# Lennart0HU/Master-Thesis-Deep-Reinforcement-Learning-DDPG-in-Home-Energy-Management

Hardware: AMD Instinct MI355X
Metric: env-steps/sec (higher is better)
Workload: dtype f32; 1 GPU; 65536 parallel shems_LU1 envs per GPU, Charger98 synthetic train table (4320 rows), 72-step episodes, mode=train; envs_per_gpu=65536, episode_len=72, mode=train

## Files before the change

master-thesis-deep-reinforcement-learning-ddpg-in-home-energy-management_amd/csrc/shems_ddpg.hip:

```cpp
#include <hip/hip_runtime.h>

#include <cstring>
#include <type_traits>

#include "philox.h"
#include "shems_internal.h"
#include "shems_adam.h"

namespace shems {

typedef float f32x16 __attribute__((ext_vector_type(16)));

#ifdef SHEMS_STAMP
__device__ unsigned long long *g_stamps = nullptr;
#define STAMP(region, i) do { if (threadIdx.x == 0 && g_stamps) { unsigned long long *sp_ = g_stamps + ((((size_t)(region) * 1024 + blockIdx.x) * 16 + (i)) * 2); \
        sp_[0] = __builtin_amdgcn_s_memtime(); sp_[1] = __builtin_amdgcn_s_memrealtime(); } } while (0)
#else
#define STAMP(region, i)
#endif

constexpr int BP = 128;
constexpr int H1N = SHEMS_L1, H2N = SHEMS_L2;
constexpr int SIN = 9, AIN = 2, CIN = 11;
constexpr int NT = 16;
// ... 25 lines not shown
constexpr int64_t WS_DAP = WS_IDX + BP;
constexpr int64_t WS_FW3C = WS_DAP + NT16 * AIN * BP;
constexpr int64_t WS_FW3A = WS_FW3C + 512;
constexpr int64_t WS_FB3 = WS_FW3A + 1024;
constexpr int64_t WS_W1T = WS_FB3 + 8;
constexpr int64_t WS_EA1 = WS_W1T + 4 * 12 * 256;
constexpr int64_t WS_SLOT0 = WS_EA1 + NQ * H1N * BP;
constexpr int64_t SL_H2 = 0;
constexpr int64_t SL_P3 = SL_H2 + H2N * BP;
constexpr int64_t SL_EP = SL_P3 + NT * 2 * BP;
constexpr int64_t SL_SIZE = SL_EP + NQ * H1N * BP;
enum { SLOT_ACTOR_T = 0, SLOT_CRITIC_T = 1, SLOT_CRITIC = 2, SLOT_ACTOR = 3, SLOT_CRITIC2 = 4, N_SLOTS = 5 };
static_assert(WS_W1T % 4 == 0 && WS_SLOT0 % 4 == 0 && SL_SIZE % 4 == 0, "16-byte aligned blocks");
__host__ __device__ inline float *w1t_of(float *ws, int net) { return ws + WS_W1T + (int64_t)net * 12 * 256; }
constexpr int64_t WS_SYNC = WS_SLOT0 + N_SLOTS * SL_SIZE;
constexpr int64_t WS_FLOATS = WS_SYNC + 96;
static_assert(WS_FLOATS == kTpWsFloats, "shems_internal.h states the workspace size for shems_gupd.hip");

__host__ __device__ inline float *slot(float *ws, int s) { return ws + WS_SLOT0 + (int64_t)s * SL_SIZE; }

template <int CTRL, int ROW_MASK>
__device__ __forceinline__ float dpp_add(float x)
{
    const int y = __builtin_amdgcn_update_dpp(0, __builtin_bit_cast(int, x), CTRL, ROW_MASK, 0xF, false);
    return x + __builtin_bit_cast(float, y);
}
__device__ __forceinline__ float wave_sum(float x)
{
    x = dpp_add<0xB1, 0xF>(x);
    x = dpp_add<0x4E, 0xF>(x);
    x = dpp_add<0x141, 0xF>(x);
// ... 230 lines not shown
    }
}

struct FwdJob {
    const float *w1t;
    const float *P;
    int in;
    int out;
    int which;
    XSrc x;
    float *H2;
    float *P3;
    const float *d3q;
    float *DAP;
    const float *W2t;
};
struct FwdArgs { FwdJob job[3]; int64_t gstride; int prep; PrepArgs pa; };
__device__ __forceinline__ void gshift(FwdJob &J, int64_t off)
{
    J.w1t = gsh(J.w1t, off); J.P = gsh(J.P, off); gshift(J.x, off); J.H2 = gsh(J.H2, off); J.P3 = gsh(J.P3, off);
    J.d3q = gsh(J.d3q, off); J.DAP = gsh(J.DAP, off);
}

template <bool QG> struct FwdShape {
    static constexpr int WST = QG ? 36 : 32;
    static constexpr int LDS = (256 * WST + W1K * 32 + W1K * W1C + 256 + 4 * 16 * 64 + 4 * 2 * 32 + (QG ? 32 * 32 + 4 * 2 * 32 : 0)) * 4;
};

template <int IN, int PREP, bool QG, bool CLONE = false, bool TILED = false>
__device__ __forceinline__ void fwd_body(const FwdJob &J, float *smem, const PrepArgs *pa, int bx, int job)
{
    typedef FwdShape<QG> SH;
    constexpr int WST = SH::WST;
    float *Wc = smem;
    float *xs = Wc + 256 * WST;
    float *w1 = xs + W1K * 32;
    float *ep = w1 + W1K * W1C;
    float *xch = ep + 256;
    float *pp = xch + 4 * 16 * 64;
    float *Mt = pp + 4 * 2 * 32;
    float *red = Mt + 32 * 32;
    const int tid = threadIdx.x, lane = tid & 63, wave = tid >> 6, li = lane & 31, lh = lane >> 5;
    constexpr int kMTiles = BP / 32;
    constexpr int kRegion = PREP == 1 ? 0 : PREP == 0 ? 1 : 3;
    (void)kRegion;
    STAMP(kRegion, 0);
    if (PREP == 1 && bx >= NT * kMTiles) {
        if (job != 0) return;
        const int duty = bx - NT * kMTiles;
        const shems_ddpg &d = pa->d;
        if (duty == 0) {
            if (tid < BP) {
                PrepRegs pr;
                prep_load<CLONE>(*pa, tid, 0, true, pr);
// ... 105 lines not shown
    STAMP(kRegion, 5);
    {
        float xv[4][4], eb[4], e0[4], e1[4];
#pragma unroll
        for (int q = 0; q < 4; ++q)
#pragma unroll
            for (int r = 0; r < 4; ++r) xv[q][r] = xch[(q * 16 + 4 * wave + r) * 64 + lane];
#pragma unroll
        for (int r = 0; r < 4; ++r) {
            const int nl = r + 8 * wave + 4 * lh;
            eb[r] = ep[nl * 3]; e0[r] = ep[nl * 3 + 1]; e1[r] = ep[nl * 3 + 2];
        }
        __builtin_amdgcn_sched_barrier(0);
        const int m = mbase + li;
        float p0 = 0.0f, p1 = 0.0f;
#pragma unroll
        for (int r = 0; r < 4; ++r) {
            const int nl = r + 8 * wave + 4 * lh, n = n0 + nl;
            const float sum = ((xv[0][r] + xv[1][r]) + xv[2][r]) + xv[3][r];
            const float h = n < H2N ? fmaxf(sum + eb[r], 0.0f) : 0.0f;
            if (J.H2 && n < H2N) J.H2[n * BP + m] = h;
            p0 = fmaf(h, e0[r], p0);
            p1 = fmaf(h, e1[r], p1);
            if (QG) Mt[nl * 32 + li] = h > 0.0f ? e0[r] * d3q : 0.0f;
        }
        p0 += __shfl_xor(p0, 32, 64);
        p1 += __shfl_xor(p1, 32, 64);
        if (lh == 0) { pp[(wave * 2 + 0) * 32 + li] = p0; pp[(wave * 2 + 1) * 32 + li] = p1; }
    }
    __syncthreads();
    STAMP(kRegion, 6);
    if (tid < 64) {
        const int o = tid >> 5, c = tid & 31;
        const float s = ((pp[(0 * 2 + o) * 32 + c] + pp[(1 * 2 + o) * 32 + c]) + pp[(2 * 2 + o) * 32 + c]) + pp[(3 * 2 + o) * 32 + c];
        J.P3[(ntile * 2 + o) * BP + mbase + c] = s;
    }
    if (!QG) return;
    STAMP(kRegion, 7);
    {
        float bq[16];
#pragma unroll
        for (int u = 0; u < 16; ++u) bq[u] = Mt[(2 * u + lh) * 32 + li];
        float da0 = 0.0f, da1 = 0.0f;
#pragma unroll
        for (int q = 0; q < 2; ++q) {
            const int kb = 64 * wave + 32 * q;
            float aq[16], wa0[16], wa1[16];
#pragma unroll
            for (int u = 0; u < 16; ++u) aq[u] = Wc[(kb + li) * WST + 2 * u + lh];
#pragma unroll
// ... 214 lines not shown
    const int job = A.prep == 1 ? (int)blockIdx.x / kPerJob : 0, bx = (int)blockIdx.x - job * kPerJob;
    FwdJob J = job == 0 ? A.job[0] : job == 1 ? A.job[1] : A.job[2];
    gshift(J, blockIdx.z * A.gstride);
    if (A.prep == 1) {
        PrepArgs pa = A.pa;
        gshift(pa.d, blockIdx.z * A.gstride); gshift(pa.ring, blockIdx.z * A.gstride); pa.seed += blockIdx.z;
        if (J.in == SIN) fwd_body<SIN, 1, false>(J, smem, &pa, bx, job); else fwd_body<CIN, 1, false>(J, smem, &pa, bx, job);
        return;
    }
    qg16_body(J, smem, bx);
}

struct EJob {
    const float *P;
    int in, out, col;
    const float *H2;
    float *EP;
    const float *W2t;
};
struct MidArgs { FwdJob fwd; EJob e[3]; int64_t gstride; int nfwd; };
constexpr int E_LDS = (NQW * BP + 32 * (NQW + 1) + NQW) * 4;

template <bool TILED = false>
__device__ __forceinline__ void e_body(const EJob &E, int b, float *smem)
{
    float *Bt = smem;
    float *At = Bt + NQW * BP;
    float *w3s = At + 32 * (NQW + 1);
    const int tid = threadIdx.x, lane = tid & 63, wave = tid >> 6, li = lane & 31, lh = lane >> 5;
    const int kt = b >> 3, nq = b & 7, nb = nq * NQW;
    const int mcol = tid & 127, half = tid >> 7;
    const float *__restrict__ P = E.P;
    const float *__restrict__ W2p = P + off_w2(E.in);
    STAMP(1, 0);
    float hv[32], wvp[8], w3v = 0.0f;
#pragma unroll
    for (int u = 0; u < 32; ++u) hv[u] = E.H2[min(nb + 2 * u + half, H2N - 1) * BP + mcol];
#pragma unroll
    for (int u = 0; u < 8; ++u) {
        const int e = u * 256 + tid, kl = e >> 6, nl = e & 63, k = kt * 32 + kl, n = nb + nl;
        if constexpr (TILED) wvp[u] = E.W2t[w2t_idx(k, n)];
        else wvp[u] = W2p[(int64_t)min(k, H1N - 1) * H2N + min(n, H2N - 1)];
    }
    w3v = P[off_w3(E.in) + min(nb + min(tid, NQW - 1), H2N - 1) * E.out + E.col];
    if (tid < NQW) w3s[tid] = nb + tid < H2N ? w3v : 0.0f;
    STAMP(1, 1);
    __syncthreads();
    STAMP(1, 2);
#pragma unroll
    for (int u = 0; u < 32; ++u) {
        const int nl = 2 * u + half;
        Bt[nl * BP + mcol] = hv[u] > 0.0f ? w3s[nl] : 0.0f;
    }
#pragma unroll
    for (int u = 0; u < 8; ++u) {
        const int e = u * 256 + tid, kl = e >> 6, nl = e & 63;
        At[kl * (NQW + 1) + nl] = wvp[u];
    }
    STAMP(1, 3);
    __syncthreads();
    STAMP(1, 4);
    f32x16 acc;
#pragma unroll
    for (int r = 0; r < 16; ++r) acc[r] = 0.0f;
    const float *pa = At + li * (NQW + 1), *pb = Bt + wave * 32 + li;
    {
        float ac[8], bc[8], an[8], bn[8];
// ... 11 lines not shown
#pragma unroll
            for (int u = 0; u < 8; ++u) acc = __builtin_amdgcn_mfma_f32_32x32x2f32(ac[u], bc[u], acc, 0, 0, 0);
#pragma unroll
            for (int u = 0; u < 8; ++u) { ac[u] = an[u]; bc[u] = bn[u]; }
        }
    }
    STAMP(1, 5);
    const int m = wave * 32 + li;
    float *D = E.EP + (int64_t)nq * H1N * BP;
#pragma unroll
    for (int r = 0; r < 16; ++r) {
        const int k = kt * 32 + (r & 3) + 8 * (r >> 2) + 4 * lh;
        if (k < H1N) D[k * BP + m] = acc[r];
    }
    STAMP(1, 6);
}

__global__ __launch_bounds__(256) __attribute__((amdgpu_waves_per_eu(1, 2))) void k_mid(MidArgs A)
{
    extern __shared__ __attribute__((aligned(16))) float smem[];
    const int64_t off = blockIdx.z * A.gstride;
    if ((int)blockIdx.x < A.nfwd) {
        FwdJob J = A.fwd;
        gshift(J, off);
        fwd_body<CIN, 0, false>(J, smem, nullptr, (int)blockIdx.x, 0);
        return;
    }
    const int e = (int)blockIdx.x - A.nfwd;
    const int set = e / (KT * NQ);
    EJob E = set == 0 ? A.e[0] : set == 1 ? A.e[1] : A.e[2];
    E.P = gsh(E.P, off); E.H2 = gsh(E.H2, off); E.EP = gsh(E.EP, off);
    e_body(E, e % (KT * NQ), smem);
}

__device__ __forceinline__ void adam_elem(const AdamCtx &c, int i, float graw)
{
    float m = c.mt[i], v = c.vt[i], p = c.p[i], t = c.target[i];
    adam_math(c, graw, m, v, p, t);
    c.mt[i] = m; c.vt[i] = v; c.p[i] = p; c.target[i] = t;
    if (c.publish) pub_store(c.publish + i, p, true);
}
template <int N>
__device__ __forceinline__ void adam_batch(const AdamCtx &c, const int (&idx)[N], const float (&g)[N])
{
    float m[N], v[N], p[N], t[N];
#pragma unroll
// ... 65 lines not shown
    const int64_t l = blockIdx.z;
    gshift(c, l * gstride);
    c.eta = critic ? hp[l].eta_crit : hp[l].eta_act;
    c.k1 = c.eta / (1.0 - c.bp1);
    c.tau = hp[l].tau;
    const int i0 = 4 * ((int)blockIdx.x * (int)blockDim.x + (int)threadIdx.x);
    if (i0 < c.n) adam_vec4(c, i0);
}

struct HeadRegs { float v[2 * NT]; float s[4]; };
static_assert(2 * NT >= NT16, "HeadRegs.v holds the actor head's NT16 partials");
__device__ __forceinline__ void head_loss_load(const shems_ddpg &d, HeadRegs &R)
{
    const float *ws = d.ws;
    const int m = threadIdx.x & 127;
    const float *Pt = slot(d.ws, SLOT_CRITIC_T) + SL_P3, *Pc = slot(d.ws, SLOT_CRITIC) + SL_P3;
#pragma unroll
    for (int i = 0; i < NT; ++i) { R.v[i] = Pt[(i * 2) * BP + m]; R.v[NT + i] = Pc[(i * 2) * BP + m]; }
    R.s[0] = ws[WS_FB3 + 1];
    R.s[1] = ws[WS_FB3 + 0];
    R.s[2] = ws[WS_R + m];
    R.s[3] = ws[WS_DONE + m];
}
__device__ __forceinline__ void head_actor_load(const shems_ddpg &d, HeadRegs &R, bool wt = false)
{
    const float *ws = d.ws;
    const int t = threadIdx.x, o = t >> 7, m = t & 127;
#pragma unroll
    for (int p = 0; p < NT16; ++p) R.v[p] = pub_load(ws + WS_DAP + (int64_t)(p * 2 + o) * BP + m, wt);
    R.s[0] = pub_load(ws + WS_API + t, wt);
    R.s[1] = R.s[2] = R.s[3] = 0.0f;
}

__device__ __forceinline__ void head_loss(const shems_ddpg &d, const HeadRegs &R, float *d3 , float *red , bool publisher,
                                          const AdamCtx *fuse)
{
    float *ws = d.ws;
    const int t = threadIdx.x, m = t & 127;
    float dq = 0.0f, diff = 0.0f;
    if (t < BP) {
        float q2 = R.s[0], q = R.s[1];
#pragma unroll
        for (int i = 0; i < NT; ++i) { q2 += R.v[i]; q += R.v[NT + i]; }
        const float y = R.s[2] + d.gamma * (1.0f - R.s[3]) * q2;
        diff = m < d.batch ? q - y : 0.0f;
        dq = 2.0f * diff / (float)d.batch;
        if (publisher) { ws[WS_Y + m] = y; ws[WS_Q + m] = q; ws[WS_D3C + m] = dq; }
    }
    d3[t] = t < BP ? dq : 0.0f;
    if (publisher) {
        const float s1 = wave_sum(diff * diff), s2 = wave_sum(dq);
        if ((t & 63) == 0) { red[t >> 6] = s1; red[4 + (t >> 6)] = s2; }
        __syncthreads();
        if (t == 0) {
            d.losses[0] = (red[0] + red[1]) / (float)d.batch;
            const float g = red[4] + red[5];
            d.grad_critic[off_b3(CIN, 1)] = g;
            if (fuse) adam_elem(*fuse, off_b3(CIN, 1), g);
        }
// ... 66 lines not shown
            const float g0 = red[0] + red[1], g1 = red[2] + red[3];
            d.grad_actor[off_b3(SIN, 2) + 0] = g0;
            d.grad_actor[off_b3(SIN, 2) + 1] = g1;
            d.losses[1] = ((red[4] + red[5]) + (red[6] + red[7])) / (2.0f * (float)d.batch);
            if (fuse) { adam_elem(*fuse, off_b3(SIN, 2), g0); adam_elem(*fuse, off_b3(SIN, 2) + 1, g1); }
        }
    }
}

struct GradArgs {
    const float *w1t;
    const float *P;
    int in, out;
    XSrc x;
    const float *H2;
    const float *w3f;
    float *grad;
    const float *E0, *E1;
    int head;
    int fuse;
    shems_ddpg dd;
    AdamCtx c;
    int64_t gstride;
    float *w2t;
};
__device__ __forceinline__ void gshift(GradArgs &B, int64_t off)
{
    B.w1t = gsh(B.w1t, off); B.P = gsh(B.P, off); gshift(B.x, off); B.H2 = gsh(B.H2, off); B.w3f = gsh(B.w3f, off);
    B.grad = gsh(B.grad, off); B.E0 = gsh(B.E0, off); B.E1 = gsh(B.E1, off); gshift(B.dd, off); gshift(B.c, off);
}
constexpr int GR_WN = 32;
enum { GR_NTW = 512 / GR_WN, GR_NW = KT * GR_NTW, GR_NG = 16, GR_GROWS = 512 / GR_NG, GR_GU = GR_GROWS / 4, GR_NR = (H1N + 3) / 4 };

constexpr int GR_PS = BP + 4;
constexpr int GR_BT = GR_WN * GR_PS;
constexpr int GR_AT = 32 * GR_PS;
constexpr int GR_LDS = (GR_BT + GR_AT + W1K * BP + W1K * 32 + AIN * BP + 2 * 32 + 8 + GR_GROWS * 3) * 4;

__device__ __forceinline__ float d2_val(float h2, float w3a, float w3b, float d3a, float d3b)
{
    const float g = fmaf(w3b, d3b, w3a * d3a);
    return h2 > 0.0f ? g : 0.0f;
}

template <int IN, int OUT> struct L1Row { float w[IN]; float b; float e[OUT][2][NQ]; float x[2][IN]; };
template <int IN, int OUT>
__device__ __forceinline__ void l1row_load(const GradArgs &A, int k, int lane, L1Row<IN, OUT> &R)
{
#pragma unroll
    for (int j = 0; j < IN; ++j) R.w[j] = A.P[j * H1N + k];
    R.b = A.P[off_b1(IN) + k];
#pragma unroll
    for (int h = 0; h < 2; ++h) {
        const int m = lane + 64 * h;
#pragma unroll
        for (int q = 0; q < NQ; ++q) {
            R.e[0][h][q] = A.E0[((int64_t)q * H1N + k) * BP + m];
// ... 43 lines not shown
    const AdamCtx *fz = A.fuse ? &A.c : nullptr;
    const bool publisher = bx == 0;
    constexpr int kRegion = OUT == 1 ? 2 : 4;
    (void)kRegion;
    STAMP(kRegion, 0);

    if (!is_w && !is_g) {
        const int k = (bx - GR_NW - GR_NG) * 4 + wave;
        HeadRegs hr;
        L1Row<IN, OUT> R;
        l1row_load<IN, OUT>(A, min(k, H1N - 1), lane, R);
        if constexpr (CLONE) head_clone_load(A.dd, hr);
        else if (A.head == 1) head_loss_load(A.dd, hr); else head_actor_load(A.dd, hr);
        STAMP(kRegion, 1);
        if constexpr (CLONE) head_clone(A.dd, hr, d3, red, false, nullptr);
        else if (A.head == 1) head_loss(A.dd, hr, d3, red, false, nullptr); else head_actor(A.dd, hr, d3, red, false, nullptr);
        __syncthreads();
        STAMP(kRegion, 2);
        if (k >= H1N) return;
        float gout[IN + 1];
        l1row_wave<IN, OUT>(R, d3, lane, gout);
        STAMP(kRegion, 3);
        float mine = 0.0f;
#pragma unroll
        for (int j = 0; j <= IN; ++j) mine = lane == j ? gout[j] : mine;
        if (lane <= IN) {
            const int e = lane < IN ? lane * H1N + k : off_b1(IN) + k;
            A.grad[e] = mine;
            if (fz) adam_elem(*fz, e, mine);
        }
        STAMP(kRegion, 4);
        return;
    }

    constexpr int HVN = GR_WN / 2;
    constexpr int WOWN = 4;
    float hv[HVN];
    int widx[WOWN];
    [[maybe_unused]] int tidx[WOWN];
    [[maybe_unused]] AdamCtx cw;
    if constexpr (TILED) {
        cw = A.c;
        cw.mt = A.w2t; cw.vt = A.w2t + W2T_TILE; cw.p = A.w2t + 2 * W2T_TILE; cw.target = A.w2t + 3 * W2T_TILE; cw.publish = nullptr;
    }
#pragma unroll
    for (int r = 0; r < WOWN; ++r) {
        widx[r] = -1;
        if constexpr (TILED) tidx[r] = -1;
    }
    AdamRegs<WOWN> ar;
    if (is_w) {
#pragma unroll
        for (int u = 0; u < HVN; ++u) hv[u] = A.H2[min(nt * GR_WN + 2 * u + half, H2N - 1) * BP + mcol];
#pragma unroll
        for (int r = 0; r < WOWN; ++r) {
            const int k = kt * 32 + 16 * (wave >> 1) + 4 * (lane >> 4) + r, n = nt * GR_WN + 16 * (wave & 1) + (lane & 15);
            widx[r] = (k < H1N && n < H2N) ? off_w2(IN) + k * H2N + n : -1;
            if constexpr (TILED) tidx[r] = (k < H1N && n < H2N) ? w2t_idx(k, n) : -1;
        }
        if constexpr (TILED) adam_load<WOWN>(cw, tidx, ar);
        else adam_load<WOWN>(A.c, widx, ar);
    }
    XRegs<IN> xr;
    f32x4 wq = {0.f, 0.f, 0.f, 0.f};
    float w3v = 0.0f;
    const int nrow0 = is_w ? nt * GR_WN : (bx - GR_NW) * GR_GROWS;
    if (is_w) {
        build_x_load<IN>(A.x, xr);
// ... 14 lines not shown
    if constexpr (CLONE) head_clone(A.dd, hr, d3, red, publisher, fz);
    else if (A.head == 1) head_loss(A.dd, hr, d3, red, publisher, fz); else head_actor(A.dd, hr, d3, red, publisher, fz);
    if (tid < 2 * 32) w3s[tid] = (tid & 1) < OUT ? w3v : 0.0f;
    STAMP(kRegion, 1);
    __syncthreads();
    STAMP(kRegion, 2);
    const float d3a = d3[mcol], d3b = d3[BP + mcol];

    if (is_w) {
        const f32x16 t = l1_tile<32>(w1, xs, 0, wave * 32, li, lh);
        {
#pragma unroll
            for (int u = 0; u < HVN; ++u) {
                const int nl = 2 * u + half;
                const float2 w = *reinterpret_cast<const float2 *>(w3s + 2 * nl);
                Bt[nl * GR_PS + mcol] = d2_val(hv[u], w.x, w.y, d3a, d3b);
            }
        }
#pragma unroll
        for (int r = 0; r < 16; ++r) At[((r & 3) + 8 * (r >> 2) + 4 * lh) * GR_PS + wave * 32 + li] = fmaxf(t[r], 0.0f);
        STAMP(kRegion, 3);
        __syncthreads();
        STAMP(kRegion, 4);
        f32x4 blk;
        {
            const int g = lane >> 4, c = lane & 15;
            const float *pa = At + (16 * (wave >> 1) + c) * GR_PS + 4 * g, *pb = Bt + (16 * (wave & 1) + c) * GR_PS + 4 * g;
            f32x4 av[8], bv[8];
#pragma unroll
            for (int q = 0; q < 8; ++q) {
                av[q] = *reinterpret_cast<const f32x4 *>(pa + 16 * q);
// ... 27 lines not shown
        const float e0a = d3[lane], e0b = d3[64 + lane], e1a = d3[BP + lane], e1b = d3[BP + 64 + lane];
        {
            float h0[GR_GU], h1[GR_GU];
#pragma unroll
            for (int u = 0; u < GR_GU; ++u) {
                const int nc = min(g * GR_GROWS + wave + 4 * u, H2N - 1);
                h0[u] = A.H2[nc * BP + lane];
                h1[u] = A.H2[nc * BP + 64 + lane];
            }
#pragma unroll
            for (int u = 0; u < GR_GU; ++u) {
                const int rl = wave + 4 * u;
                const float2 w = *reinterpret_cast<const float2 *>(w3s + 2 * rl);
                const float s0 = wave_sum(h0[u] * e0a + h1[u] * e0b);
                const float s1 = wave_sum(h0[u] * e1a + h1[u] * e1b);
                const float sb = wave_sum(d2_val(h0[u], w.x, w.y, e0a, e1a) + d2_val(h1[u], w.x, w.y, e0b, e1b));
                if (lane == 0) { gbuf[rl * 3 + 0] = sb; gbuf[rl * 3 + 1] = s0; gbuf[rl * 3 + 2] = s1; }
            }
        }
        STAMP(kRegion, 5);
        __syncthreads();
        if (tid < GR_GROWS * 3) {
            const int rl = tid / 3, c = tid - rl * 3, nn = g * GR_GROWS + rl;
            if (nn < H2N && c - 1 < OUT) {
                const int e = c == 0 ? off_b2(IN) + nn : off_w3(IN) + nn * OUT + (c - 1);
                const float v = gbuf[tid];
                A.grad[e] = v;
                if (fz) adam_elem(*fz, e, v);
            }
        }
        STAMP(kRegion, 7);
// ... 102 lines not shown
        const PrepArgs pa = A.pa;
        if (J.in == SIN) fwd_body<SIN, 1, false, false, true>(J, smem, &pa, bx, job); else fwd_body<CIN, 1, false, false, true>(J, smem, &pa, bx, job);
        return;
    }
    qg16_body<true>(J, smem, bx);
}
__global__ __launch_bounds__(256) __attribute__((amdgpu_waves_per_eu(1, 2))) void k_mid_t(MidArgs A)
{
    extern __shared__ __attribute__((aligned(16))) float smem[];
    if ((int)blockIdx.x < A.nfwd) {
        const FwdJob J = A.fwd;
        fwd_body<CIN, 0, false, false, true>(J, smem, nullptr, (int)blockIdx.x, 0);
        return;
    }
    const int e = (int)blockIdx.x - A.nfwd;
    const int set = e / (KT * NQ);
    const EJob E = set == 0 ? A.e[0] : set == 1 ? A.e[1] : A.e[2];
    e_body<true>(E, e % (KT * NQ), smem);
}
__global__ __launch_bounds__(256) __attribute__((amdgpu_waves_per_eu(1, 2))) void k_grad_t(GradArgs A)
{
    extern __shared__ __attribute__((aligned(16))) float smem[];
    if (A.in == SIN) grad_body<SIN, 2, false, true>(A, smem, (int)blockIdx.x); else grad_body<CIN, 1, false, true>(A, smem, (int)blockIdx.x);
}

constexpr int FWD_LDS = FwdShape<false>::LDS, QG_LDS = FWD_LDS > QG16_LDS ? FWD_LDS : QG16_LDS;
constexpr int MID_LDS = FWD_LDS > E_LDS ? FWD_LDS : E_LDS;
static_assert(QG_LDS <= 160 * 1024, "one workgroup's LDS");
static int set_lds_attrs()
{
// ... 86 lines not shown

static AdamCtx adam_ctx(const shems_ddpg *d, bool critic, const AdamScalars &s)
{
    const double k1 = s.eta / (1.0 - s.bp1), ic2 = 1.0 / (1.0 - s.bp2);
    return critic ? AdamCtx{d->critic, d->grad_critic, d->m_critic, d->v_critic, d->critic_t, nullptr, SHEMS_CRITIC_PARAMS, (int)CIN,
                            s.eta, s.bp1, s.bp2, s.gscale, k1, ic2, d->tau}
                  : AdamCtx{d->actor, d->grad_actor, d->m_actor, d->v_actor, d->actor_t, s.publish, SHEMS_ACTOR_PARAMS, (int)SIN,
                            s.eta, s.bp1, s.bp2, s.gscale, k1, ic2, d->tau};
}

static int actor_e_launch(const shems_ddpg *d, unsigned L, int64_t gs, hipStream_t st)
{
    float *ws = d->ws, *SA = slot(ws, SLOT_ACTOR);
    MidArgs m;
    std::memset(&m, 0, sizeof m);
    m.gstride = gs; m.nfwd = 0;
    m.e[0] = EJob{d->actor, SIN, 2, 0, SA + SL_H2, SA + SL_EP};
    m.e[1] = EJob{d->actor, SIN, 2, 1, SA + SL_H2, ws + WS_EA1};
    m.e[2] = m.e[1];
    hipLaunchKernelGGL(k_mid, dim3(2 * KT * NQ, 1, L), dim3(256), E_LDS, st, m);
    return hip_ok(hipGetLastError(), "k_mid (actor E) launch");
}

static int critic_side(const shems_ddpg *d, const shems_replay *ring, int64_t ring_len, uint64_t seed, uint32_t tick,
                       int64_t excl_pos, int64_t excl_count, unsigned L, int64_t gs, const AdamScalars *fuse, void *stream,
                       bool critic_only = false, const shems_group_w2t *t = nullptr)
{
    if (int rc = check_ddpg(d, "shems_ddpg_critic_grad", t)) return rc;
    if (!ring || !ring->s || !ring->a || !ring->r || !ring->s2 || !ring->done || ring_len < 1 || ring_len > ring->capacity)
        return set_error(SHEMS_ERR_ARG, "shems_ddpg_critic_grad: bad replay ring / length");
    if (excl_count < 0 || excl_pos < 0 || (excl_count > 0 && (ring_len != ring->capacity || excl_count >= ring_len)))
        return set_error(SHEMS_ERR_ARG, "shems_ddpg_critic_grad_ex: an exclusion window needs a full ring and 0 <= count < capacity");
    hipStream_t st = (hipStream_t)stream;
    float *ws = d->ws;
    const XSrc none{nullptr, nullptr, nullptr, nullptr, nullptr};
    const XSrc x_s2a{ws + WS_X2T, nullptr, slot(ws, SLOT_ACTOR_T) + SL_P3, d->actor_t + off_b3(SIN, 2), nullptr};
    const XSrc x_sa{ws + WS_XT, ws + WS_AT, nullptr, nullptr, nullptr};
    float *SC = slot(ws, SLOT_CRITIC), *SA = slot(ws, SLOT_ACTOR);
    FwdArgs f;
    std::memset(&f, 0, sizeof f);
    f.gstride = gs;
    const unsigned fgx = NT * (BP / 32);
    const int flds = FWD_LDS;
    f.job[0] = FwdJob{nullptr, d->actor_t, SIN, 2, 0, none, nullptr, slot(ws, SLOT_ACTOR_T) + SL_P3, nullptr, nullptr};
    f.job[1] = FwdJob{nullptr, d->critic, CIN, 1, 1, none, SC + SL_H2, SC + SL_P3, nullptr, nullptr};
    f.job[2] = FwdJob{nullptr, d->actor, SIN, 2, 2, none, SA + SL_H2, SA + SL_P3, nullptr, nullptr};
    f.prep = 1;
    f.pa = PrepArgs{*d, *ring, ring_len, seed, tick, excl_pos, excl_count};
    if (t) { f.job[0].W2t = t->actor + 3 * W2T_TILE; f.job[1].W2t = t->critic + 2 * W2T_TILE; f.job[2].W2t = t->actor + 2 * W2T_TILE; }
    if (t) hipLaunchKernelGGL(k_fwd_t, dim3((critic_only ? 2 : 3) * (fgx + 6), 1, L), dim3(256), flds, st, f);
    else hipLaunchKernelGGL(k_fwd, dim3((critic_only ? 2 : 3) * (fgx + 6), 1, L), dim3(256), flds, st, f);
    MidArgs m;
    std::memset(&m, 0, sizeof m);
    m.gstride = gs; m.nfwd = (int)fgx;
    m.fwd = FwdJob{w1t_of(ws, SLOT_CRITIC_T), d->critic_t, CIN, 1, 0, x_s2a, nullptr, slot(ws, SLOT_CRITIC_T) + SL_P3, nullptr, nullptr};
    m.e[0] = EJob{d->critic, CIN, 1, 0, SC + SL_H2, SC + SL_EP};
    m.e[1] = EJob{d->actor, SIN, 2, 0, SA + SL_H2, SA + SL_EP};
    m.e[2] = EJob{d->actor, SIN, 2, 1, SA + SL_H2, ws + WS_EA1};
    if (t) {
        m.fwd.W2t = t->critic + 3 * W2T_TILE; m.e[0].W2t = t->critic + 2 * W2T_TILE;
        m.e[1].W2t = m.e[2].W2t = t->actor + 2 * W2T_TILE;
    }
    const bool defer_ea = critic_only || (!fuse && (d->flags & SHEMS_DDPG_DEFER_ACTOR_E) != 0);
    if (t) hipLaunchKernelGGL(k_mid_t, dim3(fgx + (defer_ea ? 1 : 3) * KT * NQ, 1, L), dim3(256), MID_LDS, st, m);
    else hipLaunchKernelGGL(k_mid, dim3(fgx + (defer_ea ? 1 : 3) * KT * NQ, 1, L), dim3(256), MID_LDS, st, m);
    GradArgs g;
    std::memset(&g, 0, sizeof g);
    g.w1t = w1t_of(ws, SLOT_CRITIC); g.P = d->critic; g.in = CIN; g.out = 1; g.x = x_sa; g.H2 = SC + SL_H2; g.w3f = ws + WS_FW3C;
    g.grad = d->grad_critic; g.E0 = SC + SL_EP; g.E1 = nullptr; g.head = 1; g.fuse = fuse ? 1 : 0; g.dd = *d; g.gstride = gs;
    g.c = adam_ctx(d, true, fuse ? *fuse : AdamScalars{0, 0.5, 0.5, 1.0, nullptr});
    g.w2t = t ? t->critic : nullptr;
    if (t) hipLaunchKernelGGL(k_grad_t, dim3(GR_NW + GR_NG + GR_NR, 1, L), dim3(256), GR_LDS, st, g);
    else hipLaunchKernelGGL(k_grad, dim3(GR_NW + GR_NG + GR_NR, 1, L), dim3(256), GR_LDS, st, g);
    return hip_ok(hipGetLastError(), "ddpg critic-side launches");
}

static int actor_side(const shems_ddpg *d, unsigned L, int64_t gs, const AdamScalars *fuse, void *stream, const shems_group_w2t *t = nullptr)
{
    if (int rc = check_ddpg(d, "shems_ddpg_actor_grad", t)) return rc;
    hipStream_t st = (hipStream_t)stream;
    float *ws = d->ws;
    const XSrc x_spi{ws + WS_XT, nullptr, slot(ws, SLOT_ACTOR) + SL_P3, d->actor + off_b3(SIN, 2), ws + WS_API};
    const XSrc x_s{ws + WS_XT, nullptr, nullptr, nullptr, nullptr};
    float *C2 = slot(ws, SLOT_CRITIC2), *SA = slot(ws, SLOT_ACTOR);
    FwdArgs f;
    std::memset(&f, 0, sizeof f);
    f.gstride = gs;
    const unsigned fgx = NT16 * (BP / 32);
    f.prep = 2;
    f.job[0] = FwdJob{nullptr, d->critic, CIN, 1, 0, x_spi, nullptr, C2 + SL_P3, ws + WS_D3Q, ws + WS_DAP};
    GradArgs g;
    std::memset(&g, 0, sizeof g);
    g.w1t = w1t_of(ws, SLOT_ACTOR); g.P = d->actor; g.in = SIN; g.out = 2; g.x = x_s; g.H2 = SA + SL_H2; g.w3f = ws + WS_FW3A;
    g.grad = d->grad_actor; g.E0 = SA + SL_EP; g.E1 = ws + WS_EA1; g.head = 2; g.fuse = fuse ? 1 : 0; g.dd = *d; g.gstride = gs;
    g.c = adam_ctx(d, false, fuse ? *fuse : AdamScalars{0, 0.5, 0.5, 1.0, nullptr});
    if (t) {
        f.job[0].W2t = t->critic + 2 * W2T_TILE; g.w2t = t->actor;
        hipLaunchKernelGGL(k_fwd_t, dim3(fgx, 1, L), dim3(256), QG16_LDS, st, f);
        hipLaunchKernelGGL(k_grad_t, dim3(GR_NW + GR_NG + GR_NR, 1, L), dim3(256), GR_LDS, st, g);
        return hip_ok(hipGetLastError(), "ddpg actor-side launches");
    }
    hipLaunchKernelGGL(k_fwd, dim3(fgx, 1, L), dim3(256), QG16_LDS, st, f);
    hipLaunchKernelGGL(k_grad, dim3(GR_NW + GR_NG + GR_NR, 1, L), dim3(256), GR_LDS, st, g);
    return hip_ok(hipGetLastError(), "ddpg actor-side launches");
}

static int adam_launch(const shems_ddpg *d, bool critic, const AdamScalars &s, hipStream_t st, unsigned L, int64_t gs)
{
// ... 115 lines not shown
{
    const char *fn = "shems_ddpg_clone_update";
    if (int rc = check_adam(bp1, bp2, fn)) return rc;
    if (int rc = check_ddpg(d, fn)) return rc;
    if (!ring || !ring->s || !ring->a || !ring->r || !ring->s2 || !ring->done || ring_len < 1 || ring_len > ring->capacity)
        return set_error(SHEMS_ERR_ARG, "%s: bad replay ring / length", fn);
    if (int rc = set_lds_attrs_clone()) return rc;
    hipStream_t st = (hipStream_t)stream;
    float *ws = d->ws, *SA = slot(ws, SLOT_ACTOR);
    const XSrc none{nullptr, nullptr, nullptr, nullptr, nullptr};
    const XSrc x_s{ws + WS_XT, nullptr, nullptr, nullptr, nullptr};
    const AdamScalars sa{eta, bp1, bp2, 1.0, d_publish};
    FwdArgs f;
    std::memset(&f, 0, sizeof f);
    f.job[0] = FwdJob{nullptr, d->actor, SIN, 2, 2, none, SA + SL_H2, SA + SL_P3, nullptr, nullptr};
    f.prep = 1;
    f.pa = PrepArgs{*d, *ring, ring_len, seed, tick, 0, 0};
    hipLaunchKernelGGL(k_fwd_clone, dim3(NT * (BP / 32) + 6), dim3(256), FWD_LDS, st, f);
    if (int rc = actor_e_launch(d, 1, 0, st)) return rc;
    GradArgs g;
    std::memset(&g, 0, sizeof g);
    g.w1t = w1t_of(ws, SLOT_ACTOR); g.P = d->actor; g.in = SIN; g.out = 2; g.x = x_s; g.H2 = SA + SL_H2; g.w3f = ws + WS_FW3A;
    g.grad = d->grad_actor; g.E0 = SA + SL_EP; g.E1 = ws + WS_EA1; g.head = 3; g.fuse = 1; g.dd = *d; g.gstride = 0;
    g.c = adam_ctx(d, false, sa);
    hipLaunchKernelGGL(k_grad_clone, dim3(GR_NW + GR_NG + GR_NR), dim3(256), GR_LDS, st, g);
    return hip_ok(hipGetLastError(), "ddpg clone-update launches");
}

int shems_ddpg_critic_update(const shems_ddpg *d, const shems_replay *ring, int64_t ring_len, uint64_t seed, uint32_t tick,
                             double eta, double bp1, double bp2, void *stream)
{
    if (int rc = check_adam(bp1, bp2, "shems_ddpg_critic_update")) return rc;
    const AdamScalars sc{eta, bp1, bp2, 1.0, nullptr};
    return critic_side(d, ring, ring_len, seed, tick, 0, 0, 1, 0, &sc, stream, true);
}

int shems_ddpg_group_update(const shems_ddpg *d0, const shems_replay *ring0, const shems_group *g, int64_t ring_len, uint64_t seed,
// ... 130 lines not shown
```

master-thesis-deep-reinforcement-learning-ddpg-in-home-energy-management_amd/csrc/shems_internal.h:

```cpp
#pragma once
#include <hip/hip_runtime.h>
#include <atomic>
#include <cstdint>
#include "../../include/shems_hip.h"

namespace shems {
int set_error(int code, const char *fmt, ...);
int hip_ok(hipError_t e, const char *what);
inline int lds_optin(std::atomic<uint64_t> &mask, const void *fn, int bytes, const char *what)
{
    int dev = 0;
    if (int rc = hip_ok(hipGetDevice(&dev), "hipGetDevice")) return rc;
    const uint64_t bit = 1ull << (dev & 63);
    if (mask.load(std::memory_order_acquire) & bit) return SHEMS_OK;
    if (int rc = hip_ok(hipFuncSetAttribute(fn, hipFuncAttributeMaxDynamicSharedMemorySize, bytes), what)) return rc;
    mask.fetch_or(bit, std::memory_order_release);
    return SHEMS_OK;
}
constexpr int64_t kTpWsFloats = 1902568;
int check_view(const shems_view *v, const char *fn);
bool w2t_lookup(const float *block, shems_group_w2t *out);
int w2t_flux_guard(const float *block, const char *fn);
int adam_soft_sweep(float *p, const float *g, float *m, float *v, float *target, float *publish, int n, double eta, double bp1, double bp2,
                    double gscale, float tau, hipStream_t st);
int adam_soft_sweep_group(float *p, const float *g, float *m, float *v, float *target, int n, double eta, double bp1, double bp2, float tau,
                          int count, int64_t gstride_bytes, const shems_group_hparams *hp, bool critic, hipStream_t st);
int wide_actor_pre(const float *actor, const float *s_min, const float *s_max, int l1, int l2, const float *d_obs, int64_t m, float *d_ws,
                   float *d_part, int *n_partials, hipStream_t st);
int64_t wide_act_ws_floats(int l1, int l2, int64_t m);
int wide_actor_pre_group(const float *actor0, const float *s_min0, const float *s_max0, int64_t stride, int count, int64_t epl, int l1, int l2,
                         const float *d_obs, float *d_ws, float *d_part, int *n_partials, hipStream_t st);
int64_t wide_act_part_offset(int l1, int64_t m);
}
```

Before: 402.4 million env-steps/s.

## Pack layer-2 ReLU masks into bitwords and precompute critic Q per row

The forward kernel now emits a 32-bit mask per 32-neuron tile recording which hidden-2 activations are positive. The E and gradient kernels read one mask word instead of 16-32 float H2 values to decide gating. An extra block in the mid kernel pre-sums the critic Q so the head-loss load reads one value instead of sixteen partials. This cuts global reads in the backward stages at the cost of extra workspace, a cross-lane shuffle and an added block. The TD target in the grad head is also made non-fused to keep rounding consistent.

```diff
diff --git a/master-thesis-deep-reinforcement-learning-ddpg-in-home-energy-management_amd/csrc/shems_ddpg.hip b/master-thesis-deep-reinforcement-learning-ddpg-in-home-energy-management_amd/csrc/shems_ddpg.hip
--- a/master-thesis-deep-reinforcement-learning-ddpg-in-home-energy-management_amd/csrc/shems_ddpg.hip
+++ b/master-thesis-deep-reinforcement-learning-ddpg-in-home-energy-management_amd/csrc/shems_ddpg.hip
@@ -63,7 +63,10 @@
 static_assert(WS_W1T % 4 == 0 && WS_SLOT0 % 4 == 0 && SL_SIZE % 4 == 0, "16-byte aligned blocks");
 __host__ __device__ inline float *w1t_of(float *ws, int net) { return ws + WS_W1T + (int64_t)net * 12 * 256; }
 constexpr int64_t WS_SYNC = WS_SLOT0 + N_SLOTS * SL_SIZE;
-constexpr int64_t WS_FLOATS = WS_SYNC + 96;
+constexpr int64_t WS_MASKC = WS_SYNC + 96;
+constexpr int64_t WS_MASKA = WS_MASKC + NT * BP;
+constexpr int64_t WS_QE = WS_MASKA + NT * BP;
+constexpr int64_t WS_FLOATS = WS_QE + BP;
 static_assert(WS_FLOATS == kTpWsFloats, "shems_internal.h states the workspace size for shems_gupd.hip");
 
 __host__ __device__ inline float *slot(float *ws, int s) { return ws + WS_SLOT0 + (int64_t)s * SL_SIZE; }
@@ -324,12 +327,13 @@
     const float *d3q;
     float *DAP;
     const float *W2t;
+    uint32_t *M;
 };
 struct FwdArgs { FwdJob job[3]; int64_t gstride; int prep; PrepArgs pa; };
 __device__ __forceinline__ void gshift(FwdJob &J, int64_t off)
 {
     J.w1t = gsh(J.w1t, off); J.P = gsh(J.P, off); gshift(J.x, off); J.H2 = gsh(J.H2, off); J.P3 = gsh(J.P3, off);
-    J.d3q = gsh(J.d3q, off); J.DAP = gsh(J.DAP, off);
+    J.d3q = gsh(J.d3q, off); J.DAP = gsh(J.DAP, off); J.M = gsh(J.M, off);
 }
 
 template <bool QG> struct FwdShape {
@@ -348,6 +352,7 @@
     float *ep = w1 + W1K * W1C;
     float *xch = ep + 256;
     float *pp = xch + 4 * 16 * 64;
+    uint32_t *mk = reinterpret_cast<uint32_t *>(ep + 128);
     float *Mt = pp + 4 * 2 * 32;
     float *red = Mt + 32 * 32;
     const int tid = threadIdx.x, lane = tid & 63, wave = tid >> 6, li = lane & 31, lh = lane >> 5;
@@ -483,6 +488,7 @@
         __builtin_amdgcn_sched_barrier(0);
         const int m = mbase + li;
         float p0 = 0.0f, p1 = 0.0f;
+        uint32_t bits = 0;
 #pragma unroll
         for (int r = 0; r < 4; ++r) {
             const int nl = r + 8 * wave + 4 * lh, n = n0 + nl;
@@ -491,11 +497,13 @@
             if (J.H2 && n < H2N) J.H2[n * BP + m] = h;
             p0 = fmaf(h, e0[r], p0);
             p1 = fmaf(h, e1[r], p1);
+            bits |= (h > 0.0f ? 1u : 0u) << nl;
             if (QG) Mt[nl * 32 + li] = h > 0.0f ? e0[r] * d3q : 0.0f;
         }
         p0 += __shfl_xor(p0, 32, 64);
         p1 += __shfl_xor(p1, 32, 64);
-        if (lh == 0) { pp[(wave * 2 + 0) * 32 + li] = p0; pp[(wave * 2 + 1) * 32 + li] = p1; }
+        bits |= (uint32_t)__shfl_xor((int)bits, 32, 64);
+        if (lh == 0) { pp[(wave * 2 + 0) * 32 + li] = p0; pp[(wave * 2 + 1) * 32 + li] = p1; mk[wave * 32 + li] = bits; }
     }
     __syncthreads();
     STAMP(kRegion, 6);
@@ -503,6 +511,9 @@
         const int o = tid >> 5, c = tid & 31;
         const float s = ((pp[(0 * 2 + o) * 32 + c] + pp[(1 * 2 + o) * 32 + c]) + pp[(2 * 2 + o) * 32 + c]) + pp[(3 * 2 + o) * 32 + c];
         J.P3[(ntile * 2 + o) * BP + mbase + c] = s;
+    } else if (J.M && tid < 96) {
+        const int c = tid & 31;
+        J.M[ntile * BP + mbase + c] = (mk[c] | mk[32 + c]) | (mk[64 + c] | mk[96 + c]);
     }
     if (!QG) return;
     STAMP(kRegion, 7);
@@ -747,11 +758,11 @@
 struct EJob {
     const float *P;
     int in, out, col;
-    const float *H2;
+    const uint32_t *M;
     float *EP;
     const float *W2t;
 };
-struct MidArgs { FwdJob fwd; EJob e[3]; int64_t gstride; int nfwd; };
+struct MidArgs { FwdJob fwd; EJob e[3]; int64_t gstride; int nfwd; int ne; float *qws; };
 constexpr int E_LDS = (NQW * BP + 32 * (NQW + 1) + NQW) * 4;
 
 template <bool TILED = false>
@@ -766,9 +777,8 @@
     const float *__restrict__ P = E.P;
     const float *__restrict__ W2p = P + off_w2(E.in);
     STAMP(1, 0);
-    float hv[32], wvp[8], w3v = 0.0f;
-#pragma unroll
-    for (int u = 0; u < 32; ++u) hv[u] = E.H2[min(nb + 2 * u + half, H2N - 1) * BP + mcol];
+    float wvp[8], w3v = 0.0f;
+    const uint32_t mw0 = E.M[(2 * nq) * BP + mcol], mw1 = E.M[(2 * nq + 1) * BP + mcol];
 #pragma unroll
     for (int u = 0; u < 8; ++u) {
         const int e = u * 256 + tid, kl = e >> 6, nl = e & 63, k = kt * 32 + kl, n = nb + nl;
@@ -783,7 +793,7 @@
 #pragma unroll
     for (int u = 0; u < 32; ++u) {
         const int nl = 2 * u + half;
-        Bt[nl * BP + mcol] = hv[u] > 0.0f ? w3s[nl] : 0.0f;
+        Bt[nl * BP + mcol] = (((u < 16 ? mw0 : mw1) >> (nl & 31)) & 1u) ? w3s[nl] : 0.0f;
     }
 #pragma unroll
     for (int u = 0; u < 8; ++u) {
@@ -825,6 +835,19 @@
         if (k < H1N) D[k * BP + m] = acc[r];
     }
     STAMP(1, 6);
+}
+
+__device__ __forceinline__ void q_body(float *ws)
+{
+    const int m = min((int)threadIdx.x, BP - 1);
+    const float *Pc = slot(ws, SLOT_CRITIC) + SL_P3;
+    float v[NT];
+#pragma unroll
+    for (int i = 0; i < NT; ++i) v[i] = Pc[(i * 2) * BP + m];
+    float q = ws[WS_FB3 + 0];
+#pragma unroll
+    for (int i = 0; i < NT; ++i) q += v[i];
+    if (threadIdx.x < BP) ws[WS_QE + m] = q;
 }
 
 __global__ __launch_bounds__(256) __attribute__((amdgpu_waves_per_eu(1, 2))) void k_mid(MidArgs A)
@@ -838,9 +861,10 @@
         return;
     }
     const int e = (int)blockIdx.x - A.nfwd;
+    if (e >= A.ne) { q_body(gsh(A.qws, off)); return; }
     const int set = e / (KT * NQ);
     EJob E = set == 0 ? A.e[0] : set == 1 ? A.e[1] : A.e[2];
-    E.P = gsh(E.P, off); E.H2 = gsh(E.H2, off); E.EP = gsh(E.EP, off);
+    E.P = gsh(E.P, off); E.M = gsh(E.M, off); E.EP = gsh(E.EP, off);
     e_body(E, e % (KT * NQ), smem);
 }
 
@@ -936,11 +960,11 @@
 {
     const float *ws = d.ws;
     const int m = threadIdx.x & 127;
-    const float *Pt = slot(d.ws, SLOT_CRITIC_T) + SL_P3, *Pc = slot(d.ws, SLOT_CRITIC) + SL_P3;
-#pragma unroll
-    for (int i = 0; i < NT; ++i) { R.v[i] = Pt[(i * 2) * BP + m]; R.v[NT + i] = Pc[(i * 2) * BP + m]; }
+    const float *Pt = slot(d.ws, SLOT_CRITIC_T) + SL_P3;
+#pragma unroll
+    for (int i = 0; i < NT; ++i) R.v[i] = Pt[(i * 2) * BP + m];
     R.s[0] = ws[WS_FB3 + 1];
-    R.s[1] = ws[WS_FB3 + 0];
+    R.s[1] = ws[WS_QE + m];
     R.s[2] = ws[WS_R + m];
     R.s[3] = ws[WS_DONE + m];
 }
@@ -954,6 +978,19 @@
     R.s[1] = R.s[2] = R.s[3] = 0.0f;
 }
 
+template <bool ROWS>
+__device__ __forceinline__ float td_target(float r, float g1d, float q2)
+{
+    if constexpr (ROWS) {
+#pragma clang fp contract(off)
+        const float prod = g1d * q2;
+        return r + prod;
+    } else {
+        return fmaf(g1d, q2, r);
+    }
+}
+
+template <bool ROWS = false>
 __device__ __forceinline__ void head_loss(const shems_ddpg &d, const HeadRegs &R, float *d3 , float *red , bool publisher,
                                           const AdamCtx *fuse)
 {
@@ -961,10 +998,11 @@
     const int t = threadIdx.x, m = t & 127;
     float dq = 0.0f, diff = 0.0f;
     if (t < BP) {
-        float q2 = R.s[0], q = R.s[1];
-#pragma unroll
-        for (int i = 0; i < NT; ++i) { q2 += R.v[i]; q += R.v[NT + i]; }
-        const float y = R.s[2] + d.gamma * (1.0f - R.s[3]) * q2;
+        float q2 = R.s[0];
+        const float q = R.s[1];
+#pragma unroll
+        for (int i = 0; i < NT; ++i) q2 += R.v[i];
+        const float y = td_target<ROWS>(R.s[2], d.gamma * (1.0f - R.s[3]), q2);
         diff = m < d.batch ? q - y : 0.0f;
         dq = 2.0f * diff / (float)d.batch;
         if (publisher) { ws[WS_Y + m] = y; ws[WS_Q + m] = q; ws[WS_D3C + m] = dq; }
@@ -1061,6 +1099,7 @@
     int in, out;
     XSrc x;
     const float *H2;
+    const uint32_t *M;
     const float *w3f;
     float *grad;
     const float *E0, *E1;
@@ -1073,7 +1112,7 @@
 };
 __device__ __forceinline__ void gshift(GradArgs &B, int64_t off)
 {
-    B.w1t = gsh(B.w1t, off); B.P = gsh(B.P, off); gshift(B.x, off); B.H2 = gsh(B.H2, off); B.w3f = gsh(B.w3f, off);
+    B.w1t = gsh(B.w1t, off); B.P = gsh(B.P, off); gshift(B.x, off); B.H2 = gsh(B.H2, off); B.M = gsh(B.M, off); B.w3f = gsh(B.w3f, off);
     B.grad = gsh(B.grad, off); B.E0 = gsh(B.E0, off); B.E1 = gsh(B.E1, off); gshift(B.dd, off); gshift(B.c, off);
 }
 constexpr int GR_WN = 32;
@@ -1084,10 +1123,10 @@
 constexpr int GR_AT = 32 * GR_PS;
 constexpr int GR_LDS = (GR_BT + GR_AT + W1K * BP + W1K * 32 + AIN * BP + 2 * 32 + 8 + GR_GROWS * 3) * 4;
 
-__device__ __forceinline__ float d2_val(float h2, float w3a, float w3b, float d3a, float d3b)
+__device__ __forceinline__ float d2_val(bool on, float w3a, float w3b, float d3a, float d3b)
 {
     const float g = fmaf(w3b, d3b, w3a * d3a);
-    return h2 > 0.0f ? g : 0.0f;
+    return on ? g : 0.0f;
 }
 
 template <int IN, int OUT> struct L1Row { float w[IN]; float b; float e[OUT][2][NQ]; float x[2][IN]; };
@@ -1161,7 +1200,7 @@
         else if (A.head == 1) head_loss_load(A.dd, hr); else head_actor_load(A.dd, hr);
         STAMP(kRegion, 1);
         if constexpr (CLONE) head_clone(A.dd, hr, d3, red, false, nullptr);
-        else if (A.head == 1) head_loss(A.dd, hr, d3, red, false, nullptr); else head_actor(A.dd, hr, d3, red, false, nullptr);
+        else if (A.head == 1) head_loss<true>(A.dd, hr, d3, red, false, nullptr); else head_actor(A.dd, hr, d3, red, false, nullptr);
         __syncthreads();
         STAMP(kRegion, 2);
         if (k >= H1N) return;
@@ -1180,9 +1219,10 @@
         return;
     }
 
+    static_assert(GR_WN == 32, "a W tile's n range is one mask word");
     constexpr int HVN = GR_WN / 2;
     constexpr int WOWN = 4;
-    float hv[HVN];
+    uint32_t mw = 0;
     int widx[WOWN];
     [[maybe_unused]] int tidx[WOWN];
     [[maybe_unused]] AdamCtx cw;
@@ -1197,8 +1237,7 @@
     }
     AdamRegs<WOWN> ar;
     if (is_w) {
-#pragma unroll
-        for (int u = 0; u < HVN; ++u) hv[u] = A.H2[min(nt * GR_WN + 2 * u + half, H2N - 1) * BP + mcol];
+        mw = A.M[nt * BP + mcol];
 #pragma unroll
         for (int r = 0; r < WOWN; ++r) {
             const int k = kt * 32 + 16 * (wave >> 1) + 4 * (lane >> 4) + r, n = nt * GR_WN + 16 * (wave & 1) + (lane & 15);
@@ -1243,7 +1282,7 @@
             for (int u = 0; u < HVN; ++u) {
                 const int nl = 2 * u + half;
                 const float2 w = *reinterpret_cast<const float2 *>(w3s + 2 * nl);
-                Bt[nl * GR_PS + mcol] = d2_val(hv[u], w.x, w.y, d3a, d3b);
+                Bt[nl * GR_PS + mcol] = d2_val(((mw >> nl) & 1u) != 0, w.x, w.y, d3a, d3b);
             }
         }
 #pragma unroll
@@ -1301,7 +1340,7 @@
                 const float2 w = *reinterpret_cast<const float2 *>(w3s + 2 * rl);
                 const float s0 = wave_sum(h0[u] * e0a + h1[u] * e0b);
                 const float s1 = wave_sum(h0[u] * e1a + h1[u] * e1b);
-                const float sb = wave_sum(d2_val(h0[u], w.x, w.y, e0a, e1a) + d2_val(h1[u], w.x, w.y, e0b, e1b));
+                const float sb = wave_sum(d2_val(h0[u] > 0.0f, w.x, w.y, e0a, e1a) + d2_val(h1[u] > 0.0f, w.x, w.y, e0b, e1b));
                 if (lane == 0) { gbuf[rl * 3 + 0] = sb; gbuf[rl * 3 + 1] = s0; gbuf[rl * 3 + 2] = s1; }
             }
         }
@@ -1434,6 +1473,7 @@
         return;
     }
     const int e = (int)blockIdx.x - A.nfwd;
+    if (e >= A.ne) { q_body(A.qws); return; }
     const int set = e / (KT * NQ);
     const EJob E = set == 0 ? A.e[0] : set == 1 ? A.e[1] : A.e[2];
     e_body<true>(E, e % (KT * NQ), smem);
@@ -1550,9 +1590,10 @@
     float *ws = d->ws, *SA = slot(ws, SLOT_ACTOR);
     MidArgs m;
     std::memset(&m, 0, sizeof m);
-    m.gstride = gs; m.nfwd = 0;
-    m.e[0] = EJob{d->actor, SIN, 2, 0, SA + SL_H2, SA + SL_EP};
-    m.e[1] = EJob{d->actor, SIN, 2, 1, SA + SL_H2, ws + WS_EA1};
+    m.gstride = gs; m.nfwd = 0; m.ne = 2 * KT * NQ;
+    const uint32_t *MA = reinterpret_cast<const uint32_t *>(ws + WS_MASKA);
+    m.e[0] = EJob{d->actor, SIN, 2, 0, MA, SA + SL_EP};
+    m.e[1] = EJob{d->actor, SIN, 2, 1, MA, ws + WS_EA1};
     m.e[2] = m.e[1];
     hipLaunchKernelGGL(k_mid, dim3(2 * KT * NQ, 1, L), dim3(256), E_LDS, st, m);
     return hip_ok(hipGetLastError(), "k_mid (actor E) launch");
@@ -1581,6 +1622,8 @@
     f.job[0] = FwdJob{nullptr, d->actor_t, SIN, 2, 0, none, nullptr, slot(ws, SLOT_ACTOR_T) + SL_P3, nullptr, nullptr};
     f.job[1] = FwdJob{nullptr, d->critic, CIN, 1, 1, none, SC + SL_H2, SC + SL_P3, nullptr, nullptr};
     f.job[2] = FwdJob{nullptr, d->actor, SIN, 2, 2, none, SA + SL_H2, SA + SL_P3, nullptr, nullptr};
+    uint32_t *MC = reinterpret_cast<uint32_t *>(ws + WS_MASKC), *MA = reinterpret_cast<uint32_t *>(ws + WS_MASKA);
+    f.job[1].M = MC; f.job[2].M = MA;
     f.prep = 1;
     f.pa = PrepArgs{*d, *ring, ring_len, seed, tick, excl_pos, excl_count};
     if (t) { f.job[0].W2t = t->actor + 3 * W2T_TILE; f.job[1].W2t = t->critic + 2 * W2T_TILE; f.job[2].W2t = t->actor + 2 * W2T_TILE; }
@@ -1590,19 +1633,20 @@
     std::memset(&m, 0, sizeof m);
     m.gstride = gs; m.nfwd = (int)fgx;
     m.fwd = FwdJob{w1t_of(ws, SLOT_CRITIC_T), d->critic_t, CIN, 1, 0, x_s2a, nullptr, slot(ws, SLOT_CRITIC_T) + SL_P3, nullptr, nullptr};
-    m.e[0] = EJob{d->critic, CIN, 1, 0, SC + SL_H2, SC + SL_EP};
-    m.e[1] = EJob{d->actor, SIN, 2, 0, SA + SL_H2, SA + SL_EP};
-    m.e[2] = EJob{d->actor, SIN, 2, 1, SA + SL_H2, ws + WS_EA1};
+    m.e[0] = EJob{d->critic, CIN, 1, 0, MC, SC + SL_EP};
+    m.e[1] = EJob{d->actor, SIN, 2, 0, MA, SA + SL_EP};
+    m.e[2] = EJob{d->actor, SIN, 2, 1, MA, ws + WS_EA1};
     if (t) {
         m.fwd.W2t = t->critic + 3 * W2T_TILE; m.e[0].W2t = t->critic + 2 * W2T_TILE;
         m.e[1].W2t = m.e[2].W2t = t->actor + 2 * W2T_TILE;
     }
     const bool defer_ea = critic_only || (!fuse && (d->flags & SHEMS_DDPG_DEFER_ACTOR_E) != 0);
-    if (t) hipLaunchKernelGGL(k_mid_t, dim3(fgx + (defer_ea ? 1 : 3) * KT * NQ, 1, L), dim3(256), MID_LDS, st, m);
-    else hipLaunchKernelGGL(k_mid, dim3(fgx + (defer_ea ? 1 : 3) * KT * NQ, 1, L), dim3(256), MID_LDS, st, m);
+    m.ne = (defer_ea ? 1 : 3) * KT * NQ; m.qws = ws;
+    if (t) hipLaunchKernelGGL(k_mid_t, dim3(fgx + m.ne + 1, 1, L), dim3(256), MID_LDS, st, m);
+    else hipLaunchKernelGGL(k_mid, dim3(fgx + m.ne + 1, 1, L), dim3(256), MID_LDS, st, m);
     GradArgs g;
     std::memset(&g, 0, sizeof g);
-    g.w1t = w1t_of(ws, SLOT_CRITIC); g.P = d->critic; g.in = CIN; g.out = 1; g.x = x_sa; g.H2 = SC + SL_H2; g.w3f = ws + WS_FW3C;
+    g.w1t = w1t_of(ws, SLOT_CRITIC); g.P = d->critic; g.in = CIN; g.out = 1; g.x = x_sa; g.H2 = SC + SL_H2; g.M = MC; g.w3f = ws + WS_FW3C;
     g.grad = d->grad_critic; g.E0 = SC + SL_EP; g.E1 = nullptr; g.head = 1; g.fuse = fuse ? 1 : 0; g.dd = *d; g.gstride = gs;
     g.c = adam_ctx(d, true, fuse ? *fuse : AdamScalars{0, 0.5, 0.5, 1.0, nullptr});
     g.w2t = t ? t->critic : nullptr;
@@ -1627,7 +1671,7 @@
     f.job[0] = FwdJob{nullptr, d->critic, CIN, 1, 0, x_spi, nullptr, C2 + SL_P3, ws + WS_D3Q, ws + WS_DAP};
     GradArgs g;
     std::memset(&g, 0, sizeof g);
-    g.w1t = w1t_of(ws, SLOT_ACTOR); g.P = d->actor; g.in = SIN; g.out = 2; g.x = x_s; g.H2 = SA + SL_H2; g.w3f = ws + WS_FW3A;
+    g.w1t = w1t_of(ws, SLOT_ACTOR); g.P = d->actor; g.in = SIN; g.out = 2; g.x = x_s; g.H2 = SA + SL_H2; g.M = reinterpret_cast<const uint32_t *>(ws + WS_MASKA); g.w3f = ws + WS_FW3A;
     g.grad = d->grad_actor; g.E0 = SA + SL_EP; g.E1 = ws + WS_EA1; g.head = 2; g.fuse = fuse ? 1 : 0; g.dd = *d; g.gstride = gs;
     g.c = adam_ctx(d, false, fuse ? *fuse : AdamScalars{0, 0.5, 0.5, 1.0, nullptr});
     if (t) {
@@ -1773,13 +1817,14 @@
     FwdArgs f;
     std::memset(&f, 0, sizeof f);
     f.job[0] = FwdJob{nullptr, d->actor, SIN, 2, 2, none, SA + SL_H2, SA + SL_P3, nullptr, nullptr};
+    f.job[0].M = reinterpret_cast<uint32_t *>(ws + WS_MASKA);
     f.prep = 1;
     f.pa = PrepArgs{*d, *ring, ring_len, seed, tick, 0, 0};
     hipLaunchKernelGGL(k_fwd_clone, dim3(NT * (BP / 32) + 6), dim3(256), FWD_LDS, st, f);
     if (int rc = actor_e_launch(d, 1, 0, st)) return rc;
     GradArgs g;
     std::memset(&g, 0, sizeof g);
-    g.w1t = w1t_of(ws, SLOT_ACTOR); g.P = d->actor; g.in = SIN; g.out = 2; g.x = x_s; g.H2 = SA + SL_H2; g.w3f = ws + WS_FW3A;
+    g.w1t = w1t_of(ws, SLOT_ACTOR); g.P = d->actor; g.in = SIN; g.out = 2; g.x = x_s; g.H2 = SA + SL_H2; g.M = reinterpret_cast<const uint32_t *>(ws + WS_MASKA); g.w3f = ws + WS_FW3A;
     g.grad = d->grad_actor; g.E0 = SA + SL_EP; g.E1 = ws + WS_EA1; g.head = 3; g.fuse = 1; g.dd = *d; g.gstride = 0;
     g.c = adam_ctx(d, false, sa);
     hipLaunchKernelGGL(k_grad_clone, dim3(GR_NW + GR_NG + GR_NR), dim3(256), GR_LDS, st, g);
diff --git a/master-thesis-deep-reinforcement-learning-ddpg-in-home-energy-management_amd/csrc/shems_internal.h b/master-thesis-deep-reinforcement-learning-ddpg-in-home-energy-management_amd/csrc/shems_internal.h
--- a/master-thesis-deep-reinforcement-learning-ddpg-in-home-energy-management_amd/csrc/shems_internal.h
+++ b/master-thesis-deep-reinforcement-learning-ddpg-in-home-energy-management_amd/csrc/shems_internal.h
@@ -17,7 +17,7 @@
     mask.fetch_or(bit, std::memory_order_release);
     return SHEMS_OK;
 }
-constexpr int64_t kTpWsFloats = 1902568;
+constexpr int64_t kTpWsFloats = 1906792;
 int check_view(const shems_view *v, const char *fn);
 bool w2t_lookup(const float *block, shems_group_w2t *out);
 int w2t_flux_guard(const float *block, const char *fn);
```

New measurement: 403.3 million env-steps/s (median of 6 runs). About the same (+0.2%).
